# learning-at-home/dalle

Hardware: AMD Instinct MI355X
Metric: training samples/sec (whole node), DALL-E d_model=1024 at 1/2/4/8 MI355X (higher is better)
Workload: dtype bf16; 1 GPU; model=DALL-E d_model=1024, 24 layers, 256 text + 32x32 image tokens, preset=bench24, global_batch=128, per_gpu_batch=128, seq_len=1280, parallelism=dp1, unique_params=125648484, engine=GradSync + fused LAMB, optimizer=LAMB (32-bit moments) + global clip 4.0, grad_allreduce_dtype=fp32, grad_allreduce_algo=rccl, gemm_selection=off, reversible=no, grad_compression=none

## Files before the change

csrc/kernels/attention.hip:

```cpp
#include <cstdio>
#include <cstdlib>

#include "common.h"
#include <stdlib.h>
#include "geom.h"

#include "attn_tile.h"

namespace dalle {

__device__ __forceinline__ void rope_bwd_store_full(const RopeOut& ro, const AttnGeom& g, int bh, int s0, int t,
                                                    const f32x16& acc0, const f32x16& acc1, float scale, float* stage,
                                                    int lane) {
  const int hl = lane >> 5, c32 = lane & 31;
  const int b = bh / g.H, h = bh - b * g.H, HD = g.H * 64;
  const int q8 = lane & 7, d0 = 8 * q8;
  int pp[4];
  f32x4 c0[2], c1[2], n0[2], n1[2];
  auto load_tab = [&](int it) {
    const int tok = it * 8 + (lane >> 3);
    const int p = st2seq(g, s0 + tok);
    pp[it] = p;
    const int pc = p < 0 ? 0 : p;
    const float* cp = ro.cosT + (size_t)pc * 64 + d0;
    const float* sp = ro.sinT + (size_t)pc * 64 + d0;
    c0[it & 1] = *reinterpret_cast<const f32x4*>(cp);
    c1[it & 1] = *reinterpret_cast<const f32x4*>(cp + 4);
    n0[it & 1] = *reinterpret_cast<const f32x4*>(sp);
    n1[it & 1] = *reinterpret_cast<const f32x4*>(sp + 4);
  };
  load_tab(0);
  load_tab(1);
#pragma unroll
  for (int dt = 0; dt < 2; ++dt) {
    const f32x16& acc = dt ? acc1 : acc0;
#pragma unroll
    for (int gq = 0; gq < 4; ++gq) {
      const int ch = (8 * dt + 2 * gq + hl) ^ (c32 & 15);
      *reinterpret_cast<f32x4*>(stage + c32 * 64 + 4 * ch) = f32x4{acc[4 * gq], acc[4 * gq + 1], acc[4 * gq + 2], acc[4 * gq + 3]};
    }
  }
  __builtin_amdgcn_s_waitcnt(0xC07F);
  __builtin_amdgcn_wave_barrier();
#pragma unroll
  for (int it = 0; it < 4; ++it) {
    const int tok = it * 8 + (lane >> 3), sl = it & 1;
    const f32x4 lo = *reinterpret_cast<const f32x4*>(stage + tok * 64 + 4 * ((2 * q8) ^ (tok & 15)));
    const f32x4 hi = *reinterpret_cast<const f32x4*>(stage + tok * 64 + 4 * ((2 * q8 + 1) ^ (tok & 15)));
    const float x[8] = {lo[0], lo[1], lo[2], lo[3], hi[0], hi[1], hi[2], hi[3]};
    const float c[8] = {c0[sl][0], c0[sl][1], c0[sl][2], c0[sl][3], c1[sl][0], c1[sl][1], c1[sl][2], c1[sl][3]};
    const float sn[8] = {n0[sl][0], n0[sl][1], n0[sl][2], n0[sl][3], n1[sl][0], n1[sl][1], n1[sl][2], n1[sl][3]};
    const int p = pp[it];
    if (it + 2 < 4) load_tab(it + 2);
    float y[8];
#pragma unroll
    for (int i = 0; i < 8; i += 2) {
      const float a0 = x[i] * scale, a1 = x[i + 1] * scale;
      y[i] = a0 * c[i] + a1 * sn[i + 1];
      y[i + 1] = a1 * c[i + 1] + a0 * sn[i];
    }
    if (p >= 0) *reinterpret_cast<s16x8*>(ro.dqkv + ((size_t)b * g.n + p) * (3 * HD) + t * HD + h * 64 + d0) = pack8(y);
  }
  __builtin_amdgcn_wave_barrier();
}

constexpr float RESCALE_THR = 8.0f;

__device__ __forceinline__ float half_max(float x) {
  const auto r = __builtin_amdgcn_permlane32_swap(__float_as_uint(x), __float_as_uint(x), false, false);
  return fmaxf(__uint_as_float(r[0]), __uint_as_float(r[1]));
}
__device__ __forceinline__ float half_sum(float x) {
  const auto r = __builtin_amdgcn_permlane32_swap(__float_as_uint(x), __float_as_uint(x), false, false);
  return __uint_as_float(r[0]) + __uint_as_float(r[1]);
}

struct SoftmaxState {
  float m = NEG_BIG;
  float lsum = 0.f;
  f32x16 o0 = {}, o1 = {};
};

template <int NT>
__device__ __forceinline__ void fwd_tiles(SoftmaxState& st, const __bf16* const (&Ks)[NT], const __bf16* const (&Vs)[NT],
                                          const int (&kt)[NT], const bf16x8 (&qf)[4], const AttnGeom& g, int qb, int qs,
                                          int lane) {
  const int hl = lane >> 5, c32 = lane & 31;
  constexpr float THR_RAW = RESCALE_THR / LOG2E;
  f32x16 s[NT];
#pragma unroll
  for (int j = 0; j < NT; ++j) {
    s[j] = f32x16{};
#pragma unroll
    for (int ss = 0; ss < 4; ++ss) s[j] = MFMA32(row_operand(Ks[j], ss, c32, hl), qf[ss], s[j]);
// ... 128 lines not shown
        const int c = lane + 64 * j, row = c >> 3, col = (c & 7) * 8;
        *reinterpret_cast<s16x8*>(P + lds_idx(row, col)) = kr[j];
        *reinterpret_cast<s16x8*>(P + TILE + lds_idx(row, col)) = vr[j];
      }
      if (t < qb) load_loc(t + 1);
      __builtin_amdgcn_s_waitcnt(0xC07F);
      __builtin_amdgcn_wave_barrier();
      const __bf16* const Ks[1] = {P};
      const __bf16* const Vs[1] = {P + TILE};
      const int kt[1] = {t};
      fwd_tiles<1>(st, Ks, Vs, kt, qf, g, qb, qs, lane);
      __builtin_amdgcn_wave_barrier();
    }
  }

  if (!active) return;
  const float ltot = half_sum(st.lsum);
  const float inv = 1.0f / ltot;
  lse[(size_t)bh * g.Np + qs] = st.m * LOG2E + log2f(ltot);
  __bf16* Os = smem + wave * (2 * TILE);
#pragma unroll
  for (int dt = 0; dt < 2; ++dt) {
    const f32x16& o = dt ? st.o1 : st.o0;
#pragma unroll
    for (int gq = 0; gq < 4; ++gq) {
      float f[4];
#pragma unroll
      for (int i = 0; i < 4; ++i) f[i] = o[4 * gq + i] * inv;
      *reinterpret_cast<s16x4*>(Os + lds_idx(c32, 32 * dt + 8 * gq + 4 * hl)) = pack4(f);
    }
  }
  __builtin_amdgcn_s_waitcnt(0xC07F);
  __builtin_amdgcn_wave_barrier();
#pragma unroll
  for (int i = 0; i < 4; ++i) {
    const int row = 8 * i + (lane >> 3), col = (lane & 7) * 8;
    const s16x8 v = *reinterpret_cast<const s16x8*>(Os + lds_idx(row, col));
    const int p = st2seq(g, qb * 32 + row);
    if (p >= 0) *reinterpret_cast<s16x8*>(out + ((size_t)b * g.n + p) * (g.H * 64) + h * 64 + col) = v;
  }
}

__global__ __launch_bounds__(256) void attn_delta_kernel(const __bf16* __restrict__ dout, const __bf16* __restrict__ out,
                                                         float* __restrict__ delta, AttnGeom g, int BH) {
  const long gid = (long)blockIdx.x * blockDim.x + threadIdx.x;
  const int chunk = gid & 7;
  const long row_g = gid >> 3;
  if (row_g >= (long)BH * g.Np) return;
  const int bh = row_g / g.Np, srow = row_g - (long)bh * g.Np;
  const int off = tok_row(g, srow);
  float acc = 0.f;
  if (off >= 0) {
    float fd[8], fo[8];
    unpack8(ld_tok(tok_base(dout, g, bh), off, chunk * 8), fd);
    unpack8(ld_tok(tok_base(out, g, bh), off, chunk * 8), fo);
#pragma unroll
    for (int i = 0; i < 8; ++i) acc = fmaf(fd[i], fo[i], acc);
  }
  acc += __shfl_xor(acc, 1, 64);
  acc += __shfl_xor(acc, 2, 64);
  acc += __shfl_xor(acc, 4, 64);
  if (chunk == 0) delta[row_g] = acc;
}

__device__ __forceinline__ void dq_tile(f32x16& dq0, f32x16& dq1, const __bf16* Ks, const __bf16* Vs, int tile,
                                        const bf16x8 (&qf)[4], const bf16x8 (&dof)[4], float lq, float dl,
                                        const AttnGeom& g, int qb, int qs, int lane) {
  const int hl = lane >> 5, c32 = lane & 31;
  f32x16 s = {}, dp = {};
#pragma unroll
  for (int ss = 0; ss < 4; ++ss) {
    s = MFMA32(row_operand(Ks, ss, c32, hl), qf[ss], s);
    dp = MFMA32(row_operand(Vs, ss, c32, hl), dof[ss], dp);
  }
#pragma unroll
  for (int r = 0; r < 16; ++r) s[r] = fast_exp2(fmaf(s[r], LOG2E, -lq)) * (dp[r] - dl);
  if (!tile_full(g, qb, tile)) {
    const uint32_t mh = key_mask(g, qs, tile) >> (4 * hl);
#pragma unroll
    for (int r = 0; r < 16; ++r) s[r] = mask_bit(mh, r) ? s[r] : 0.f;
  }
  const bf16x8 d0 = cvt8(s, 0), d1 = cvt8(s, 8);
  dq0 = MFMA32(tr_operand(Ks, 0, 0, lane), d0, dq0);
  dq0 = MFMA32(tr_operand(Ks, 1, 0, lane), d1, dq0);
  dq1 = MFMA32(tr_operand(Ks, 0, 1, lane), d0, dq1);
  dq1 = MFMA32(tr_operand(Ks, 1, 1, lane), d1, dq1);
}

template <int MINB, bool FUSE_LOCAL, bool PREFETCH_LOCAL = false>
__global__ __launch_bounds__(256, MINB) void attn_bwd_dq_kernel(const __bf16* __restrict__ Q, const __bf16* __restrict__ Kt,
                                                             const __bf16* __restrict__ V, const __bf16* __restrict__ dout,
                                                             const __bf16* __restrict__ out, const float* __restrict__ lse,
                                                             float* __restrict__ delta, __bf16* __restrict__ dQ, AttnGeom g,
                                                             RopeOut ro, int delta_ready) {
  __shared__ __attribute__((aligned(16))) __bf16 smem[2 * 2 * 2 * TILE];
  __shared__ float fstats[FUSE_LOCAL ? 4 : 1][2][32];
  __shared__ float dsh[4][32];
  int grp, bh;
  xcd_remap(grp, bh);
  const int tid = threadIdx.x, wave = tid >> 6, lane = tid & 63, hl = lane >> 5;
  const int nqb = g.Np >> 5, ntext = g.Tp >> 5;
  const int qb0 = grp * 4;
  const int qb = qb0 + wave;
  const int qb_last = min(qb0 + 3, nqb - 1);
  const bool active = qb < nqb;
  const size_t base = (size_t)bh * g.Np * 64;
  const __bf16* dob = tok_base(dout, g, bh);
  const __bf16* outb = tok_base(out, g, bh);

  const int n_text = qb_last < ntext ? qb_last + 1 : ntext;
  const int my_text_end = active ? min(qb + 1, ntext) : 0;
  const int qs = qb * 32 + (lane & 31);
  const int qrow = active ? qs : 0;
  bf16x8 qf[4], dof[4];
  float dl = 0.f;
  {
  __bf16* Ps = smem + wave * (2 * TILE);
  float dpart[4];
  s16x8 qv[4], dv[4], ov[4];
  int toff[4];
#pragma unroll
  for (int j = 0; j < 4; ++j) {
    const int c = lane + 64 * j, row = c >> 3, col = (c & 7) * 8;
    const int srow = (active ? qb * 32 : 0) + row;
    toff[j] = tok_row(g, srow);
    const int safe = toff[j] < 0 ? 0 : toff[j];
    qv[j] = *reinterpret_cast<const s16x8*>(Q + base + (size_t)srow * 64 + col);
    dv[j] = *reinterpret_cast<const s16x8*>(dob + safe + col);
    ov[j] = *reinterpret_cast<const s16x8*>(outb + safe + col);
  }
#pragma unroll
  for (int j = 0; j < 4; ++j) {
    const int c = lane + 64 * j, row = c >> 3, col = (c & 7) * 8;
    if (toff[j] < 0) dv[j] = s16x8{};
    *reinterpret_cast<s16x8*>(Ps + lds_idx(row, col)) = qv[j];
    *reinterpret_cast<s16x8*>(Ps + TILE + lds_idx(row, col)) = dv[j];
    float fd[8], fo[8];
    unpack8(dv[j], fd);
    unpack8(ov[j], fo);
    dpart[j] = 0.f;
#pragma unroll
    for (int i = 0; i < 8; ++i) dpart[j] = fmaf(fd[i], fo[i], dpart[j]);
  }
  if (!delta_ready) {
#pragma unroll
    for (int j = 0; j < 4; ++j) {
      dpart[j] += __shfl_xor(dpart[j], 1, 64);
      dpart[j] += __shfl_xor(dpart[j], 2, 64);
      dpart[j] += __shfl_xor(dpart[j], 4, 64);
      const int row = 8 * j + (lane >> 3);
      if ((lane & 7) == 0) {
        dsh[wave][row] = dpart[j];
        if (active) delta[(size_t)bh * g.Np + qb * 32 + row] = dpart[j];
      }
    }
  }
  __builtin_amdgcn_s_waitcnt(0xC07F);
  __builtin_amdgcn_wave_barrier();
#pragma unroll
  for (int s2 = 0; s2 < 4; ++s2) {
    qf[s2] = row_operand(Ps, s2, lane & 31, hl);
    dof[s2] = row_operand(Ps + TILE, s2, lane & 31, hl);
  }
  dl = delta_ready ? delta[(size_t)bh * g.Np + qrow] : dsh[wave][lane & 31];
  __builtin_amdgcn_s_waitcnt(0xC07F);
  __syncthreads();
  }
  const float lq = lse[(size_t)bh * g.Np + qrow];
  f32x16 dq0 = {}, dq1 = {};
  const bool has_local = active && qb >= ntext;
  const int lo = has_local ? local_lo_tile(g, qb) : 0;
  s16x8 kr[4], vr[4];
  auto load_loc = [&](int t) {
#pragma unroll
    for (int j = 0; j < 4; ++j) {
      const int c = lane + 64 * j, row = c >> 3, col = (c & 7) * 8;
      const size_t off = base + (size_t)(t * 32 + row) * 64 + col;
      kr[j] = *reinterpret_cast<const s16x8*>(Kt + off);
      vr[j] = *reinterpret_cast<const s16x8*>(V + off);
    }
  };
  if (has_local && PREFETCH_LOCAL) load_loc(lo);

  {
  const int st_row = tid >> 3, st_col = (tid & 7) * 8;
  const int st_off = lds_idx(st_row, st_col);
  const int npairs = (n_text + 1) >> 1;
  s16x8 sreg[4];
  auto load_pair = [&](int pi) {
// ... 12 lines not shown
  };
  load_pair(0);
  store_pair(0);
  __syncthreads();
  for (int pi = 0; pi < npairs; ++pi) {
    const bool more = pi + 1 < npairs;
    if (more) load_pair(pi + 1);
    const __bf16* S0 = smem + (pi & 1) * (4 * TILE);
    const int ta = 2 * pi, tb = 2 * pi + 1;
    if (ta < my_text_end) dq_tile(dq0, dq1, S0, S0 + 2 * TILE, ta, qf, dof, lq, dl, g, qb, qs, lane);
    if (tb < my_text_end) dq_tile(dq0, dq1, S0 + TILE, S0 + 3 * TILE, tb, qf, dof, lq, dl, g, qb, qs, lane);
    if (more) store_pair((pi + 1) & 1);
    __syncthreads();
  }
  }

  if (has_local) {
    __bf16* P = smem + wave * (2 * TILE);
    if (!PREFETCH_LOCAL) load_loc(lo);
    for (int t = lo; t <= qb; ++t) {
#pragma unroll
      for (int j = 0; j < 4; ++j) {
        const int c = lane + 64 * j, row = c >> 3, col = (c & 7) * 8;
        *reinterpret_cast<s16x8*>(P + lds_idx(row, col)) = kr[j];
        *reinterpret_cast<s16x8*>(P + TILE + lds_idx(row, col)) = vr[j];
      }
      if (t < qb) load_loc(t + 1);
      __builtin_amdgcn_s_waitcnt(0xC07F);
      __builtin_amdgcn_wave_barrier();
      dq_tile(dq0, dq1, P, P + TILE, t, qf, dof, lq, dl, g, qb, qs, lane);
      __builtin_amdgcn_wave_barrier();
    }
  }
  if (FUSE_LOCAL && active && qb >= ntext && ro.dqkv) {
    __bf16* P = smem + wave * (2 * TILE);
    const int c32 = lane & 31;
    bf16x8 kf[4], vf[4];
#pragma unroll
    for (int s2 = 0; s2 < 4; ++s2) {
      kf[s2] = ld16(P + lds_idx(c32, 16 * s2 + 8 * hl));
      vf[s2] = ld16(P + TILE + lds_idx(c32, 16 * s2 + 8 * hl));
    }
    __builtin_amdgcn_s_waitcnt(0xC07F);
    __builtin_amdgcn_wave_barrier();
#pragma unroll
    for (int s2 = 0; s2 < 4; ++s2) {
      *reinterpret_cast<bf16x8*>(P + lds_idx(c32, 16 * s2 + 8 * hl)) = qf[s2];
      *reinterpret_cast<bf16x8*>(P + TILE + lds_idx(c32, 16 * s2 + 8 * hl)) = dof[s2];
    }
    if (hl == 0) {
      fstats[FUSE_LOCAL ? wave : 0][0][c32] = lq;
      fstats[FUSE_LOCAL ? wave : 0][1][c32] = dl;
    }
    __builtin_amdgcn_s_waitcnt(0xC07F);
    __builtin_amdgcn_wave_barrier();
    const float(*st)[32] = fstats[FUSE_LOCAL ? wave : 0];
    const int ks = qb * 32 + c32;
    f32x16 sc = {}, dp = {};
#pragma unroll
    for (int s2 = 0; s2 < 4; ++s2) {
      sc = MFMA32(row_operand(P, s2, c32, hl), kf[s2], sc);
      dp = MFMA32(row_operand(P + TILE, s2, c32, hl), vf[s2], dp);
    }
    f32x16 ds;
#pragma unroll
    for (int r = 0; r < 16; ++r) {
      const int ql = acc_row(r, hl);
      const float pr = fast_exp2(fmaf(sc[r], LOG2E, -st[0][ql]));
      sc[r] = pr;
      ds[r] = pr * (dp[r] - st[1][ql]);
    }
    const uint32_t mh = query_mask(g, ks, qb) >> (4 * hl);
#pragma unroll
    for (int r = 0; r < 16; ++r) {
      const bool on = mask_bit(mh, r);
      sc[r] = on ? sc[r] : 0.f;
      ds[r] = on ? ds[r] : 0.f;
    }
    const bf16x8 p0 = cvt8(sc, 0), p1 = cvt8(sc, 8);
    const bf16x8 e0 = cvt8(ds, 0), e1 = cvt8(ds, 8);
    f32x16 dk0 = {}, dk1 = {}, dv0 = {}, dv1 = {};
    dv0 = MFMA32(tr_operand(P + TILE, 0, 0, lane), p0, dv0);
    dv0 = MFMA32(tr_operand(P + TILE, 1, 0, lane), p1, dv0);
    dv1 = MFMA32(tr_operand(P + TILE, 0, 1, lane), p0, dv1);
    dv1 = MFMA32(tr_operand(P + TILE, 1, 1, lane), p1, dv1);
    dk0 = MFMA32(tr_operand(P, 0, 0, lane), e0, dk0);
    dk0 = MFMA32(tr_operand(P, 1, 0, lane), e1, dk0);
    dk1 = MFMA32(tr_operand(P, 0, 1, lane), e0, dk1);
    dk1 = MFMA32(tr_operand(P, 1, 1, lane), e1, dk1);
    float* stage = reinterpret_cast<float*>(P);
    rope_bwd_store_full(ro, g, bh, qb * 32, 1, dk0, dk1, 1.0f, stage, lane);
    rope_bwd_store_full(ro, g, bh, qb * 32, 2, dv0, dv1, 1.0f, stage, lane);
  }
  __syncthreads();

  if (!active) return;
  if (ro.dqkv) {
    float* stage = reinterpret_cast<float*>(smem) + wave * 2048;
    rope_bwd_store_full(ro, g, bh, qb * 32, 0, dq0, dq1, ro.qscale, stage, lane);
    return;
  }
  __bf16* qp = dQ + base + (size_t)qs * 64;
#pragma unroll
  for (int dt = 0; dt < 2; ++dt) {
    const f32x16& o = dt ? dq1 : dq0;
#pragma unroll
    for (int gq = 0; gq < 4; ++gq) {
      float f[4];
#pragma unroll
      for (int i = 0; i < 4; ++i) f[i] = o[4 * gq + i];
      *reinterpret_cast<s16x4*>(qp + 32 * dt + 8 * gq + 4 * hl) = pack4(f);
    }
  }
}

template <int MINB>
__global__ __launch_bounds__(256, MINB) void attn_bwd_dkdv_kernel(const __bf16* __restrict__ Q, const __bf16* __restrict__ Kt,
                                                               const __bf16* __restrict__ V, const __bf16* __restrict__ dout,
                                                               const float* __restrict__ lse, const float* __restrict__ delta,
                                                               __bf16* __restrict__ dK, __bf16* __restrict__ dV, AttnGeom g,
                                                               RopeOut ro) {
  __shared__ __attribute__((aligned(16))) __bf16 smem[4 * 2 * TILE];
  __shared__ float stats[4][2][32];
  int grp, bh;
  xcd_remap(grp, bh);
  const int tid = threadIdx.x, wave = tid >> 6, lane = tid & 63, hl = lane >> 5, c32 = lane & 31;
  const int nkb = g.Np >> 5, ntext = g.Tp >> 5;
  const int kb = ntext + grp * 4 + wave;
  if (kb >= nkb) return;
  const size_t base = (size_t)bh * g.Np * 64;
  const __bf16* dob = tok_base(dout, g, bh);
  const int ks = kb * 32 + c32;
  const int q_hi = local_hi_qtile(g, kb);
  bf16x8 kf[4], vf[4];
  {
    const __bf16* kp = Kt + base + (size_t)ks * 64 + 8 * hl;
    const __bf16* vp = V + base + (size_t)ks * 64 + 8 * hl;
#pragma unroll
    for (int s = 0; s < 4; ++s) { kf[s] = ld16(kp + 16 * s); vf[s] = ld16(vp + 16 * s); }
  }
  __bf16* Qs = smem + wave * (2 * TILE);
  __bf16* Ds = Qs + TILE;
  s16x8 qr[4], dr[4];
  float sv = 0.f;
  auto load_tile = [&](int qt) {
#pragma unroll
    for (int j = 0; j < 4; ++j) {
      const int c = lane + 64 * j, row = c >> 3, col = (c & 7) * 8;
      const size_t off = base + (size_t)(qt * 32 + row) * 64 + col;
      qr[j] = *reinterpret_cast<const s16x8*>(Q + off);
      dr[j] = ld_tok(dob, tok_row(g, qt * 32 + row), col);
    }
    sv = (hl ? delta : lse)[(size_t)bh * g.Np + qt * 32 + c32];
  };
  f32x16 dk0 = {}, dk1 = {}, dv0 = {}, dv1 = {};
  load_tile(kb);
  for (int qt = kb; qt <= q_hi; ++qt) {
#pragma unroll
    for (int j = 0; j < 4; ++j) {
      const int c = lane + 64 * j, row = c >> 3, col = (c & 7) * 8;
      *reinterpret_cast<s16x8*>(Qs + lds_idx(row, col)) = qr[j];
      *reinterpret_cast<s16x8*>(Ds + lds_idx(row, col)) = dr[j];
    }
    stats[wave][hl][c32] = sv;
    if (qt < q_hi) load_tile(qt + 1);
    __builtin_amdgcn_s_waitcnt(0xC07F);
    __builtin_amdgcn_wave_barrier();
    f32x16 sc = {}, dp = {};
#pragma unroll
    for (int ss = 0; ss < 4; ++ss) {
      sc = MFMA32(row_operand(Qs, ss, c32, hl), kf[ss], sc);
      dp = MFMA32(row_operand(Ds, ss, c32, hl), vf[ss], dp);
    }
    f32x16 ds;
#pragma unroll
    for (int r = 0; r < 16; ++r) {
      const int ql = acc_row(r, hl);
      const float pr = fast_exp2(fmaf(sc[r], LOG2E, -stats[wave][0][ql]));
      sc[r] = pr;
      ds[r] = pr * (dp[r] - stats[wave][1][ql]);
    }
    if (!tile_full(g, qt, kb)) {
      const uint32_t mh = query_mask(g, ks, qt) >> (4 * hl);
#pragma unroll
      for (int r = 0; r < 16; ++r) {
        const bool on = mask_bit(mh, r);
        sc[r] = on ? sc[r] : 0.f;
        ds[r] = on ? ds[r] : 0.f;
      }
    }
    const bf16x8 p0 = cvt8(sc, 0), p1 = cvt8(sc, 8);
    const bf16x8 d0 = cvt8(ds, 0), d1 = cvt8(ds, 8);
    dv0 = MFMA32(tr_operand(Ds, 0, 0, lane), p0, dv0);
    dv0 = MFMA32(tr_operand(Ds, 1, 0, lane), p1, dv0);
    dv1 = MFMA32(tr_operand(Ds, 0, 1, lane), p0, dv1);
    dv1 = MFMA32(tr_operand(Ds, 1, 1, lane), p1, dv1);
    dk0 = MFMA32(tr_operand(Qs, 0, 0, lane), d0, dk0);
    dk0 = MFMA32(tr_operand(Qs, 1, 0, lane), d1, dk0);
    dk1 = MFMA32(tr_operand(Qs, 0, 1, lane), d0, dk1);
    dk1 = MFMA32(tr_operand(Qs, 1, 1, lane), d1, dk1);
    __builtin_amdgcn_wave_barrier();
  }
  if (ro.dqkv) {
    float* stage = reinterpret_cast<float*>(Qs);
    rope_bwd_store_full(ro, g, bh, kb * 32, 1, dk0, dk1, 1.0f, stage, lane);
    rope_bwd_store_full(ro, g, bh, kb * 32, 2, dv0, dv1, 1.0f, stage, lane);
    return;
  }
  __bf16* kp = dK + base + (size_t)ks * 64;
  __bf16* vp = dV + base + (size_t)ks * 64;
#pragma unroll
  for (int dt = 0; dt < 2; ++dt) {
    const f32x16& a = dt ? dk1 : dk0;
    const f32x16& c = dt ? dv1 : dv0;
#pragma unroll
    for (int gq = 0; gq < 4; ++gq) {
      float fa[4], fc[4];
#pragma unroll
      for (int i = 0; i < 4; ++i) { fa[i] = a[4 * gq + i]; fc[i] = c[4 * gq + i]; }
      *reinterpret_cast<s16x4*>(kp + 32 * dt + 8 * gq + 4 * hl) = pack4(fa);
      *reinterpret_cast<s16x4*>(vp + 32 * dt + 8 * gq + 4 * hl) = pack4(fc);
    }
  }
}

template <int MINB, int QT = 2>
__global__ __launch_bounds__(256, MINB) void attn_bwd_dkdv_text_kernel(const __bf16* __restrict__ Q, const __bf16* __restrict__ Kt,
                                                                    const __bf16* __restrict__ V, const __bf16* __restrict__ dout,
                                                                    const float* __restrict__ lse, const float* __restrict__ delta,
                                                                    __bf16* __restrict__ dK, __bf16* __restrict__ dV, AttnGeom g,
                                                                    RopeOut ro) {
  static_assert(QT == 2 || QT == 4, "QT");
  __shared__ __attribute__((aligned(16))) __bf16 smem[2 * QT * 2 * TILE];
  __shared__ float stats[2][QT][2][32];
  int grp, bh;
  xcd_remap(grp, bh);
  const int tid = threadIdx.x, wave = tid >> 6, lane = tid & 63, hl = lane >> 5, c32 = lane & 31;
  const int nqb = g.Np >> 5, ntext = g.Tp >> 5;
  const int kb0 = grp * 2;
  const bool tail = QT == 4 && kb0 + 1 >= ntext;
  const int kb = tail ? kb0 : kb0 + (wave & 1), par = tail ? wave : wave >> 1;
  const bool active = kb < ntext;
  const size_t base = (size_t)bh * g.Np * 64;
  const __bf16* dob = tok_base(dout, g, bh);
  const int ks = kb * 32 + c32;
  bf16x8 kf[4], vf[4];
  {
    const int krow = active ? ks : 0;
    const __bf16* kp = Kt + base + (size_t)krow * 64 + 8 * hl;
    const __bf16* vp = V + base + (size_t)krow * 64 + 8 * hl;
#pragma unroll
    for (int s = 0; s < 4; ++s) { kf[s] = ld16(kp + 16 * s); vf[s] = ld16(vp + 16 * s); }
  }
  const int nsteps = (nqb - kb0 + QT - 1) / QT;
  const int st_row = (tid & 255) >> 3, st_col = (tid & 7) * 8;
  const int st_off = lds_idx(st_row, st_col);
  s16x8 sreg[2 * QT];
  float sl = 0.f;
  auto load_step = [&](int i) {
#pragma unroll
    for (int pp = 0; pp < QT; ++pp) {
      const int qt = min(kb0 + QT * i + pp, nqb - 1);
      const size_t off = base + (size_t)(qt * 32 + st_row) * 64 + st_col;
      sreg[2 * pp] = *reinterpret_cast<const s16x8*>(Q + off);
      sreg[2 * pp + 1] = ld_tok(dob, tok_row(g, qt * 32 + st_row), st_col);
    }
    if (tid < QT * 64) {
      const int pp = tid >> 6, which = (tid >> 5) & 1, r = tid & 31;
      const int qt = min(kb0 + QT * i + pp, nqb - 1);
      const float* src = which ? delta : lse;
      sl = src[(size_t)bh * g.Np + qt * 32 + r];
    }
  };
  auto store_step = [&](int buf) {
#pragma unroll
    for (int pp = 0; pp < QT; ++pp) {
      __bf16* T0 = smem + (buf * QT + pp) * (2 * TILE);
      *reinterpret_cast<s16x8*>(T0 + st_off) = sreg[2 * pp];
      *reinterpret_cast<s16x8*>(T0 + TILE + st_off) = sreg[2 * pp + 1];
    }
    if (tid < QT * 64) stats[buf][tid >> 6][(tid >> 5) & 1][tid & 31] = sl;
  };
  f32x16 dk0 = {}, dk1 = {}, dv0 = {}, dv1 = {};
  if (nsteps > 0) {
    load_step(0);
    store_step(0);
  }
  __builtin_amdgcn_s_waitcnt(0x0F70);
  __syncthreads();
  auto scores = [&](const __bf16* Qs, const __bf16* Ds, f32x16& sc, f32x16& dp) {
    sc = f32x16{};
    dp = f32x16{};
#pragma unroll
    for (int ss = 0; ss < 4; ++ss) {
      sc = MFMA32(row_operand(Qs, ss, c32, hl), kf[ss], sc);
      dp = MFMA32(row_operand(Ds, ss, c32, hl), vf[ss], dp);
    }
  };
  auto probs = [&](int buf, int tt, int qt, f32x16& sc, f32x16& dp) {
#pragma unroll
    for (int r = 0; r < 16; ++r) {
      const int ql = acc_row(r, hl);
      const float pr = fast_exp2(fmaf(sc[r], LOG2E, -stats[buf][tt][0][ql]));
      sc[r] = pr;
      dp[r] = pr * (dp[r] - stats[buf][tt][1][ql]);
    }
    if (!tile_full(g, qt, kb)) {
      const uint32_t mh = query_mask(g, ks, qt) >> (4 * hl);
#pragma unroll
      for (int r = 0; r < 16; ++r) {
        const bool on = mask_bit(mh, r);
        sc[r] = on ? sc[r] : 0.f;
        dp[r] = on ? dp[r] : 0.f;
      }
    }
  };
  auto accum = [&](const __bf16* Qs, const __bf16* Ds, const f32x16& sc, const f32x16& ds) {
    const bf16x8 p0 = cvt8(sc, 0), p1 = cvt8(sc, 8);
    const bf16x8 d0 = cvt8(ds, 0), d1 = cvt8(ds, 8);
    dv0 = MFMA32(tr_operand(Ds, 0, 0, lane), p0, dv0);
    dv0 = MFMA32(tr_operand(Ds, 1, 0, lane), p1, dv0);
    dv1 = MFMA32(tr_operand(Ds, 0, 1, lane), p0, dv1);
    dv1 = MFMA32(tr_operand(Ds, 1, 1, lane), p1, dv1);
    dk0 = MFMA32(tr_operand(Qs, 0, 0, lane), d0, dk0);
    dk0 = MFMA32(tr_operand(Qs, 1, 0, lane), d1, dk0);
    dk1 = MFMA32(tr_operand(Qs, 0, 1, lane), d0, dk1);
    dk1 = MFMA32(tr_operand(Qs, 1, 1, lane), d1, dk1);
  };
  for (int i = 0; i < nsteps; ++i) {
    const bool more = i + 1 < nsteps;
    if (more) load_step(i + 1);
    const int buf = i & 1;
#pragma unroll
    for (int u = 0; u < QT / 2; ++u) {
      const int tt = tail ? par : par + 2 * u;
      const int qt = kb0 + QT * i + tt;
      if (active && qt < nqb && qt >= kb && !(tail && u > 0)) {
        const __bf16* Qs = smem + (buf * QT + tt) * (2 * TILE);
        f32x16 sc, dp;
        scores(Qs, Qs + TILE, sc, dp);
        probs(buf, tt, qt, sc, dp);
        accum(Qs, Qs + TILE, sc, dp);
      }
    }
    if (more) store_step((i + 1) & 1);
    __syncthreads();
  }
  float* red = reinterpret_cast<float*>(smem);
  if (par != 0) {
    const int slot = tail ? wave - 1 : (wave & 1);
#pragma unroll
    for (int r = 0; r < 16; ++r) {
      red[(slot * 64 + r) * 64 + lane] = dk0[r];
      red[(slot * 64 + 16 + r) * 64 + lane] = dk1[r];
      red[(slot * 64 + 32 + r) * 64 + lane] = dv0[r];
      red[(slot * 64 + 48 + r) * 64 + lane] = dv1[r];
    }
  }
  __syncthreads();
  if (par == 0 && active) {
    const int s0 = tail ? 0 : (wave & 1), s1 = tail ? 3 : s0 + 1;
    for (int sl2 = s0; sl2 < s1; ++sl2) {
      const float* mine = red + sl2 * 64 * 64;
#pragma unroll
      for (int r = 0; r < 16; ++r) {
        dk0[r] += mine[r * 64 + lane];
        dk1[r] += mine[(16 + r) * 64 + lane];
        dv0[r] += mine[(32 + r) * 64 + lane];
        dv1[r] += mine[(48 + r) * 64 + lane];
      }
    }
    if (ro.dqkv) {
      __builtin_amdgcn_s_waitcnt(0xC07F);
      __builtin_amdgcn_wave_barrier();
      float* stage = red + (wave & 1) * 64 * 64;
      rope_bwd_store_full(ro, g, bh, kb * 32, 1, dk0, dk1, 1.0f, stage, lane);
      rope_bwd_store_full(ro, g, bh, kb * 32, 2, dv0, dv1, 1.0f, stage, lane);
    } else {
      __bf16* kp = dK + base + (size_t)ks * 64;
      __bf16* vp = dV + base + (size_t)ks * 64;
#pragma unroll
      for (int dt = 0; dt < 2; ++dt) {
        const f32x16& a = dt ? dk1 : dk0;
        const f32x16& c = dt ? dv1 : dv0;
#pragma unroll
        for (int gq = 0; gq < 4; ++gq) {
          float fa[4], fc[4];
#pragma unroll
          for (int i = 0; i < 4; ++i) {
            fa[i] = a[4 * gq + i];
            fc[i] = c[4 * gq + i];
          }
          *reinterpret_cast<s16x4*>(kp + 32 * dt + 8 * gq + 4 * hl) = pack4(fa);
          *reinterpret_cast<s16x4*>(vp + 32 * dt + 8 * gq + 4 * hl) = pack4(fc);
        }
      }
    }
  }
}

void attn_fwd(const void* q, const void* k, const void* v, void* out, float* lse, const AttnGeom& g, int BH, hipStream_t st) {
  dim3 grid((g.Np / 32 + 3) / 4, BH);
  hipLaunchKernelGGL((attn_fwd_kernel<3, false>), grid, dim3(256), 0, st, (const __bf16*)q, (const __bf16*)k,
                     (const __bf16*)v, (__bf16*)out, lse, g);
}

bool attn_bwd_fused_ok(const AttnGeom& g, bool rope_out, bool has_freqs);
void attn_bwd_fused_launch(const void* q, const void* k, const void* v, const void* dout, const void* out, const float* lse,
                           const AttnGeom& g, int BH, hipStream_t st, const RopeOut& ro, const RotSpec& rsp);

void attn_bwd(const void* q, const void* k, const void* v, const void* out, const void* dout, const float* lse,
              float* delta, void* dq, void* dk, void* dv, const AttnGeom& g, int BH, hipStream_t st,
              const float* cosT, const float* sinT, void* dqkv, float qscale, const float* rotf, int rot_nl, int rot_np,
              float rot_img_text_pos, float rot_text_axial) {
  const RopeOut ro{cosT, sinT, static_cast<__bf16*>(dqkv), qscale};
  if (attn_bwd_fused_ok(g, dqkv != nullptr, rotf != nullptr)) {
    attn_bwd_fused_launch(q, k, v, dout, out, lse, g, BH, st, ro, RotSpec{rotf, rot_nl, rot_np, rot_img_text_pos, rot_text_axial});
    return;
  }
  dim3 grid((g.Np / 32 + 3) / 4, BH);
  const bool fuse_local = dqkv != nullptr && (g.pattern == 1 || g.pattern == 2);
  const int ntext = g.Tp / 32, nimg = g.Np / 32 - ntext;
  if (fuse_local)
    hipLaunchKernelGGL((attn_bwd_dq_kernel<3, true, false>), grid, dim3(256), 0, st, (const __bf16*)q, (const __bf16*)k,
                       (const __bf16*)v, (const __bf16*)dout, (const __bf16*)out, lse, delta, (__bf16*)dq, g, ro, 0);
  else
    hipLaunchKernelGGL((attn_bwd_dq_kernel<3, false, false>), grid, dim3(256), 0, st, (const __bf16*)q, (const __bf16*)k,
                       (const __bf16*)v, (const __bf16*)dout, (const __bf16*)out, lse, delta, (__bf16*)dq, g, ro, 0);
  hipLaunchKernelGGL((attn_bwd_dkdv_text_kernel<2, 4>), dim3((ntext + 1) / 2, BH), dim3(256), 0, st, (const __bf16*)q,
                     (const __bf16*)k, (const __bf16*)v, (const __bf16*)dout, lse, delta, (__bf16*)dk, (__bf16*)dv, g, ro);
  if (!fuse_local)
    hipLaunchKernelGGL((attn_bwd_dkdv_kernel<2>), dim3((nimg + 3) / 4, BH), dim3(256), 0, st, (const __bf16*)q,
                       (const __bf16*)k, (const __bf16*)v, (const __bf16*)dout, lse, delta, (__bf16*)dk, (__bf16*)dv, g, ro);
}

}
```

csrc/kernels/attn_tile.h:

```cpp
#pragma once
#include "common.h"
#include "geom.h"

namespace dalle {

__device__ __forceinline__ int swz(int r) { return (((r >> 1) & 1) << 2) | ((r >> 2) & 3); }
__device__ __forceinline__ int lds_idx(int r, int col) { return r * 64 + ((((col >> 3) ^ swz(r)) << 3) | (col & 7)); }
constexpr int TILE = 32 * 64;

__device__ __forceinline__ void dma_tile(const __bf16* src_rows, __bf16* tile, int wave, int lane) {
  const int row = 8 * wave + (lane >> 3);
  const __bf16* gp = src_rows + (size_t)row * 64 + (((lane & 7) ^ swz(row)) << 3);
  __builtin_amdgcn_global_load_lds((const void __attribute__((address_space(1)))*)gp,
                                   (void __attribute__((address_space(3)))*)(tile + 512 * wave), 16, 0, 0);
}
__device__ __forceinline__ void dma_tile_wave(const __bf16* src_rows, __bf16* tile, int lane) {
#pragma unroll
  for (int piece = 0; piece < 4; ++piece) dma_tile(src_rows, tile, piece, lane);
}
constexpr int WAIT_VM0 = 0x0F70;

__device__ __forceinline__ float fast_exp2(float x) { return __builtin_amdgcn_exp2f(x); }

__device__ __forceinline__ int st2seq(const AttnGeom& g, int s) {
  if (s < g.T) return s;
  if (s < g.Tp) return -1;
  const int kst = s - g.Tp;
  const int k = (g.pattern == 2) ? ((kst & (g.S - 1)) << g.logS) + (kst >> g.logS) : kst;
  const int p = g.T + k;
  return p < g.n ? p : -1;
}

__device__ __forceinline__ const __bf16* tok_base(const __bf16* x, const AttnGeom& g, int bh) {
  const int b = bh / g.H, h = bh - b * g.H;
  return x + (size_t)b * g.n * (g.H * 64) + h * 64;
}
__device__ __forceinline__ int tok_row(const AttnGeom& g, int s) {
  const int k = s - g.Tp;
  const int kk = (g.pattern == 2) ? ((k & (g.S - 1)) << g.logS) + (k >> g.logS) : k;
  const int p = s < g.Tp ? (s < g.T ? s : -1) : (g.T + kk < g.n ? g.T + kk : -1);
  return p < 0 ? -1 : p * (g.H * 64);
}
__device__ __forceinline__ s16x8 ld_tok(const __bf16* __restrict__ xb, int row_off, int col) {
  return row_off < 0 ? s16x8{} : *reinterpret_cast<const s16x8*>(xb + row_off + col);
}

__device__ __forceinline__ uint32_t range_bits(int lo, int hi) {
  lo = max(lo, 0);
  hi = min(hi, 31);
  if (hi < lo) return 0u;
  const uint32_t upto = hi == 31 ? 0xffffffffu : ((1u << (hi + 1)) - 1u);
  return upto & ~((1u << lo) - 1u);
}

__device__ __forceinline__ uint32_t key_mask(const AttnGeom& g, int qs, int kt) {
  const int k0 = kt * 32;
  if (qs < g.Tp) return range_bits(0, qs - k0);
  if (k0 < g.Tp) return range_bits(0, g.T - 1 - k0);
  const int qk = qs - g.Tp, kk0 = k0 - g.Tp;
  if (g.pattern == 0) return range_bits(0, qk - kk0);
  const int qr = qk >> g.logS;
  if (g.pattern != 3) return range_bits((qr << g.logS) - kk0, qk - kk0);
  const int qc = qk & (g.S - 1);
  const int c_lo = max(0, qc - g.K + 1);
  const int rows = g.S >= 32 ? 1 : (32 >> g.logS);
  uint32_t m = 0u;
  for (int i = 0; i < rows; ++i) {
    const int kr = (kk0 >> g.logS) + i;
    if (kr > qr - g.K && kr <= qr) m |= range_bits((kr << g.logS) + c_lo - kk0, (kr << g.logS) + qc - kk0);
  }
  return m;
}

__device__ __forceinline__ uint32_t query_mask(const AttnGeom& g, int ks, int qt) {
  const int q0 = qt * 32;
  if (ks < g.Tp) {
    if (q0 < g.Tp) return range_bits(ks - q0, 31);
    return ks < g.T ? 0xffffffffu : 0u;
  }
  if (q0 < g.Tp) return 0u;
  const int kk = ks - g.Tp, qk0 = q0 - g.Tp;
  if (g.pattern == 0) return range_bits(kk - qk0, 31);
  const int kr = kk >> g.logS;
  if (g.pattern != 3) return range_bits(kk - qk0, ((kr + 1) << g.logS) - 1 - qk0);
  const int kc = kk & (g.S - 1);
  const int c_hi = min(g.S - 1, kc + g.K - 1);
  const int rows = g.S >= 32 ? 1 : (32 >> g.logS);
  uint32_t m = 0u;
  for (int i = 0; i < rows; ++i) {
    const int qr = (qk0 >> g.logS) + i;
    if (qr >= kr && qr < kr + g.K) m |= range_bits((qr << g.logS) + kc - qk0, (qr << g.logS) + c_hi - qk0);
  }
  return m;
}

__device__ __forceinline__ bool tile_full(const AttnGeom& g, int qt, int kt) {
  const int ntext = g.Tp >> 5;
  if (kt < ntext) {
    if (kt * 32 + 31 >= g.T) return false;
    return qt >= ntext || kt < qt;
  }
  return g.pattern == 0 && qt >= ntext && kt < qt;
}

__device__ __forceinline__ void xcd_remap(int& grp, int& bh) {
  const int ng = gridDim.x, BH = gridDim.y;
  if (BH & 7) { grp = blockIdx.x; bh = blockIdx.y; return; }
  const int L = blockIdx.x + blockIdx.y * ng;
  const int x = L & 7, j = L >> 3;
  bh = x + 8 * (j / ng);
  grp = j - (j / ng) * ng;
}

__device__ __forceinline__ int local_lo_tile(const AttnGeom& g, int qb) {
  const int kq0 = qb * 32 - g.Tp;
  int lo;
  if (g.pattern == 0) lo = 0;
  else if (g.pattern == 3) lo = max(0, (kq0 >> g.logS) - (g.K - 1)) << g.logS;
  else lo = (kq0 >> g.logS) << g.logS;
  return (g.Tp + lo) >> 5;
}

__device__ __forceinline__ int local_hi_qtile(const AttnGeom& g, int kb) {
  const int kk1 = kb * 32 + 31 - g.Tp;
// ... 58 lines not shown
```

Baseline: 318.6 samples/s.

## Precompute tile row positions and 32-bit byte offsets in attention backward kernels

Adds a TilePos/RopeRows helper that works out the sequence positions for a tile once, from a wave-uniform start, and stores precomputed 32-bit byte offsets. These replace the per-row st2seq/tok_row calls and 64-bit address arithmetic in the rope stores, the output writes and the dout loads. It also loads the Q tile by DMA in the dq kernel, applies the mask inside the exp so masked entries skip work, unrolls the mask loops with a fixed bound, and uses readfirstlane for wave-uniform values. A host check rejects shapes whose offsets would overflow 32 bits. The goal is lower integer/VALU and addressing overhead in the attention backward pass, which is only a small part of whole-step training.

```diff
diff --git a/csrc/kernels/attention.hip b/csrc/kernels/attention.hip
--- a/csrc/kernels/attention.hip
+++ b/csrc/kernels/attention.hip
@@ -1,5 +1,7 @@
 #include <cstdio>
 #include <cstdlib>
+#include <stdexcept>
+#include <string>
 
 #include "common.h"
 #include <stdlib.h>
@@ -9,57 +11,72 @@
 
 namespace dalle {
 
-__device__ __forceinline__ void rope_bwd_store_full(const RopeOut& ro, const AttnGeom& g, int bh, int s0, int t,
+struct RopeRows {
+  uint32_t tab[4];
+  uint32_t dst[4];
+};
+__device__ __forceinline__ RopeRows rope_rows(const AttnGeom& g, int s0, int lane) {
+  const TilePos tp = tile_pos(g, s0, lane);
+  const uint32_t q8 = lane & 7, row_bytes = 3u * g.H * 64u * 2u;
+  RopeRows rr;
+#pragma unroll
+  for (int it = 0; it < 4; ++it) {
+    const int p = tp.p[it];
+    rr.tab[it] = (uint32_t)(p < 0 ? 0 : p) * 256u + 32u * q8;
+    rr.dst[it] = p < 0 ? ~0u : (uint32_t)p * row_bytes + 16u * q8;
+  }
+  return rr;
+}
+
+template <bool SCALE>
+__device__ __forceinline__ void rope_bwd_store_full(const RopeOut& ro, const AttnGeom& g, int bh, int t, const RopeRows& rr,
                                                     const f32x16& acc0, const f32x16& acc1, float scale, float* stage,
                                                     int lane) {
   const int hl = lane >> 5, c32 = lane & 31;
   const int b = bh / g.H, h = bh - b * g.H, HD = g.H * 64;
-  const int q8 = lane & 7, d0 = 8 * q8;
-  int pp[4];
+  const int q8 = lane & 7, l3 = lane >> 3;
+  const char* cosb = reinterpret_cast<const char*>(ro.cosT);
+  const char* sinb = reinterpret_cast<const char*>(ro.sinT);
+  char* dstb = reinterpret_cast<char*>(ro.dqkv + ((size_t)b * g.n * 3 + t) * HD + h * 64);
   f32x4 c0[2], c1[2], n0[2], n1[2];
   auto load_tab = [&](int it) {
-    const int tok = it * 8 + (lane >> 3);
-    const int p = st2seq(g, s0 + tok);
-    pp[it] = p;
-    const int pc = p < 0 ? 0 : p;
-    const float* cp = ro.cosT + (size_t)pc * 64 + d0;
-    const float* sp = ro.sinT + (size_t)pc * 64 + d0;
+    const char* cp = cosb + rr.tab[it];
+    const char* sp = sinb + rr.tab[it];
     c0[it & 1] = *reinterpret_cast<const f32x4*>(cp);
-    c1[it & 1] = *reinterpret_cast<const f32x4*>(cp + 4);
+    c1[it & 1] = *reinterpret_cast<const f32x4*>(cp + 16);
     n0[it & 1] = *reinterpret_cast<const f32x4*>(sp);
-    n1[it & 1] = *reinterpret_cast<const f32x4*>(sp + 4);
+    n1[it & 1] = *reinterpret_cast<const f32x4*>(sp + 16);
   };
   load_tab(0);
   load_tab(1);
+  const int wbase = c32 * 64 + 4 * (hl ^ (c32 & 15));
 #pragma unroll
   for (int dt = 0; dt < 2; ++dt) {
     const f32x16& acc = dt ? acc1 : acc0;
 #pragma unroll
-    for (int gq = 0; gq < 4; ++gq) {
-      const int ch = (8 * dt + 2 * gq + hl) ^ (c32 & 15);
-      *reinterpret_cast<f32x4*>(stage + c32 * 64 + 4 * ch) = f32x4{acc[4 * gq], acc[4 * gq + 1], acc[4 * gq + 2], acc[4 * gq + 3]};
-    }
+    for (int gq = 0; gq < 4; ++gq)
+      *reinterpret_cast<f32x4*>(stage + (wbase ^ (4 * (8 * dt + 2 * gq)))) = f32x4{acc[4 * gq], acc[4 * gq + 1], acc[4 * gq + 2], acc[4 * gq + 3]};
   }
   __builtin_amdgcn_s_waitcnt(0xC07F);
   __builtin_amdgcn_wave_barrier();
+  const int rbase = l3 * 64 + 4 * ((2 * q8) ^ l3);
 #pragma unroll
   for (int it = 0; it < 4; ++it) {
-    const int tok = it * 8 + (lane >> 3), sl = it & 1;
-    const f32x4 lo = *reinterpret_cast<const f32x4*>(stage + tok * 64 + 4 * ((2 * q8) ^ (tok & 15)));
-    const f32x4 hi = *reinterpret_cast<const f32x4*>(stage + tok * 64 + 4 * ((2 * q8 + 1) ^ (tok & 15)));
+    const int sl = it & 1, rd = it * 512 + (rbase ^ (32 * (it & 1)));
+    const f32x4 lo = *reinterpret_cast<const f32x4*>(stage + rd);
+    const f32x4 hi = *reinterpret_cast<const f32x4*>(stage + (rd ^ 4));
     const float x[8] = {lo[0], lo[1], lo[2], lo[3], hi[0], hi[1], hi[2], hi[3]};
     const float c[8] = {c0[sl][0], c0[sl][1], c0[sl][2], c0[sl][3], c1[sl][0], c1[sl][1], c1[sl][2], c1[sl][3]};
     const float sn[8] = {n0[sl][0], n0[sl][1], n0[sl][2], n0[sl][3], n1[sl][0], n1[sl][1], n1[sl][2], n1[sl][3]};
-    const int p = pp[it];
     if (it + 2 < 4) load_tab(it + 2);
     float y[8];
 #pragma unroll
     for (int i = 0; i < 8; i += 2) {
-      const float a0 = x[i] * scale, a1 = x[i + 1] * scale;
+      const float a0 = SCALE ? x[i] * scale : x[i], a1 = SCALE ? x[i + 1] * scale : x[i + 1];
       y[i] = a0 * c[i] + a1 * sn[i + 1];
       y[i + 1] = a1 * c[i + 1] + a0 * sn[i];
     }
-    if (p >= 0) *reinterpret_cast<s16x8*>(ro.dqkv + ((size_t)b * g.n + p) * (3 * HD) + t * HD + h * 64 + d0) = pack8(y);
+    if (rr.dst[it] != ~0u) *reinterpret_cast<s16x8*>(dstb + rr.dst[it]) = pack8(y);
   }
   __builtin_amdgcn_wave_barrier();
 }
@@ -254,12 +271,14 @@
   }
   __builtin_amdgcn_s_waitcnt(0xC07F);
   __builtin_amdgcn_wave_barrier();
+  const TilePos tp = tile_pos(g, qb * 32, lane);
+  char* ob = reinterpret_cast<char*>(out + (size_t)b * g.n * (g.H * 64) + h * 64);
+  const uint32_t row_bytes = g.H * 64 * 2;
 #pragma unroll
   for (int i = 0; i < 4; ++i) {
     const int row = 8 * i + (lane >> 3), col = (lane & 7) * 8;
     const s16x8 v = *reinterpret_cast<const s16x8*>(Os + lds_idx(row, col));
-    const int p = st2seq(g, qb * 32 + row);
-    if (p >= 0) *reinterpret_cast<s16x8*>(out + ((size_t)b * g.n + p) * (g.H * 64) + h * 64 + col) = v;
+    if (tp.p[i] >= 0) *reinterpret_cast<s16x8*>(ob + ((uint32_t)tp.p[i] * row_bytes + 2 * col)) = v;
   }
 }
 
@@ -318,9 +337,13 @@
   __shared__ __attribute__((aligned(16))) __bf16 smem[2 * 2 * 2 * TILE];
   __shared__ float fstats[FUSE_LOCAL ? 4 : 1][2][32];
   __shared__ float dsh[4][32];
+  if (FUSE_LOCAL) {
+    __builtin_assume(g.pattern == 1 || g.pattern == 2);
+    __builtin_assume(ro.dqkv != nullptr);
+  }
   int grp, bh;
   xcd_remap(grp, bh);
-  const int tid = threadIdx.x, wave = tid >> 6, lane = tid & 63, hl = lane >> 5;
+  const int tid = threadIdx.x, wave = __builtin_amdgcn_readfirstlane(tid >> 6), lane = tid & 63, hl = lane >> 5;
   const int nqb = g.Np >> 5, ntext = g.Tp >> 5;
   const int qb0 = grp * 4;
   const int qb = qb0 + wave;
@@ -339,23 +362,22 @@
   {
   __bf16* Ps = smem + wave * (2 * TILE);
   float dpart[4];
-  s16x8 qv[4], dv[4], ov[4];
-  int toff[4];
+  s16x8 dv[4], ov[4];
+  const int srow0 = active ? qb * 32 : 0;
+  dma_tile_wave(Q + base + (size_t)srow0 * 64, Ps, lane);
+  const TilePos tp = tile_pos(g, srow0, lane);
+  const uint32_t row_bytes = g.H * 64 * 2;
+#pragma unroll
+  for (int j = 0; j < 4; ++j) {
+    const uint32_t off = (uint32_t)max(tp.p[j], 0) * row_bytes + 16 * (lane & 7);
+    dv[j] = *reinterpret_cast<const s16x8*>(reinterpret_cast<const char*>(dob) + off);
+    ov[j] = *reinterpret_cast<const s16x8*>(reinterpret_cast<const char*>(outb) + off);
+  }
+  __builtin_amdgcn_sched_barrier(0);
 #pragma unroll
   for (int j = 0; j < 4; ++j) {
     const int c = lane + 64 * j, row = c >> 3, col = (c & 7) * 8;
-    const int srow = (active ? qb * 32 : 0) + row;
-    toff[j] = tok_row(g, srow);
-    const int safe = toff[j] < 0 ? 0 : toff[j];
-    qv[j] = *reinterpret_cast<const s16x8*>(Q + base + (size_t)srow * 64 + col);
-    dv[j] = *reinterpret_cast<const s16x8*>(dob + safe + col);
-    ov[j] = *reinterpret_cast<const s16x8*>(outb + safe + col);
-  }
-#pragma unroll
-  for (int j = 0; j < 4; ++j) {
-    const int c = lane + 64 * j, row = c >> 3, col = (c & 7) * 8;
-    if (toff[j] < 0) dv[j] = s16x8{};
-    *reinterpret_cast<s16x8*>(Ps + lds_idx(row, col)) = qv[j];
+    if (tp.p[j] < 0) dv[j] = s16x8{};
     *reinterpret_cast<s16x8*>(Ps + TILE + lds_idx(row, col)) = dv[j];
     float fd[8], fo[8];
     unpack8(dv[j], fd);
@@ -364,19 +386,18 @@
 #pragma unroll
     for (int i = 0; i < 8; ++i) dpart[j] = fmaf(fd[i], fo[i], dpart[j]);
   }
-  if (!delta_ready) {
-#pragma unroll
-    for (int j = 0; j < 4; ++j) {
-      dpart[j] += __shfl_xor(dpart[j], 1, 64);
-      dpart[j] += __shfl_xor(dpart[j], 2, 64);
-      dpart[j] += __shfl_xor(dpart[j], 4, 64);
-      const int row = 8 * j + (lane >> 3);
-      if ((lane & 7) == 0) {
-        dsh[wave][row] = dpart[j];
-        if (active) delta[(size_t)bh * g.Np + qb * 32 + row] = dpart[j];
-      }
-    }
-  }
+#pragma unroll
+  for (int j = 0; j < 4; ++j) {
+    dpart[j] += __shfl_xor(dpart[j], 1, 64);
+    dpart[j] += __shfl_xor(dpart[j], 2, 64);
+    dpart[j] += __shfl_xor(dpart[j], 4, 64);
+    const int row = 8 * j + (lane >> 3);
+    if ((lane & 7) == 0) {
+      dsh[wave][row] = dpart[j];
+      if (!delta_ready && active) delta[(size_t)bh * g.Np + qb * 32 + row] = dpart[j];
+    }
+  }
+  __builtin_amdgcn_s_waitcnt(WAIT_VM0);
   __builtin_amdgcn_s_waitcnt(0xC07F);
   __builtin_amdgcn_wave_barrier();
 #pragma unroll
@@ -455,9 +476,11 @@
       __builtin_amdgcn_wave_barrier();
     }
   }
+  RopeRows rr = {};
+  if (active && ro.dqkv) rr = rope_rows(g, qb * 32, fresh_lane());
   if (FUSE_LOCAL && active && qb >= ntext && ro.dqkv) {
     __bf16* P = smem + wave * (2 * TILE);
-    const int c32 = lane & 31;
+    const int lane = fresh_lane(), hl = lane >> 5, c32 = lane & 31;
     bf16x8 kf[4], vf[4];
 #pragma unroll
     for (int s2 = 0; s2 < 4; ++s2) {
@@ -485,20 +508,14 @@
       sc = MFMA32(row_operand(P, s2, c32, hl), kf[s2], sc);
       dp = MFMA32(row_operand(P + TILE, s2, c32, hl), vf[s2], dp);
     }
+    const uint32_t mh = query_mask(g, ks, qb) >> (4 * hl);
     f32x16 ds;
 #pragma unroll
     for (int r = 0; r < 16; ++r) {
       const int ql = acc_row(r, hl);
-      const float pr = fast_exp2(fmaf(sc[r], LOG2E, -st[0][ql]));
+      const float pr = mask_bit(mh, r) ? fast_exp2(fmaf(sc[r], LOG2E, -st[0][ql])) : 0.f;
       sc[r] = pr;
       ds[r] = pr * (dp[r] - st[1][ql]);
-    }
-    const uint32_t mh = query_mask(g, ks, qb) >> (4 * hl);
-#pragma unroll
-    for (int r = 0; r < 16; ++r) {
-      const bool on = mask_bit(mh, r);
-      sc[r] = on ? sc[r] : 0.f;
-      ds[r] = on ? ds[r] : 0.f;
     }
     const bf16x8 p0 = cvt8(sc, 0), p1 = cvt8(sc, 8);
     const bf16x8 e0 = cvt8(ds, 0), e1 = cvt8(ds, 8);
@@ -512,15 +529,15 @@
     dk1 = MFMA32(tr_operand(P, 0, 1, lane), e0, dk1);
     dk1 = MFMA32(tr_operand(P, 1, 1, lane), e1, dk1);
     float* stage = reinterpret_cast<float*>(P);
-    rope_bwd_store_full(ro, g, bh, qb * 32, 1, dk0, dk1, 1.0f, stage, lane);
-    rope_bwd_store_full(ro, g, bh, qb * 32, 2, dv0, dv1, 1.0f, stage, lane);
+    rope_bwd_store_full<false>(ro, g, bh, 1, rr, dk0, dk1, 1.0f, stage, lane);
+    rope_bwd_store_full<false>(ro, g, bh, 2, rr, dv0, dv1, 1.0f, stage, lane);
   }
   __syncthreads();
 
   if (!active) return;
   if (ro.dqkv) {
     float* stage = reinterpret_cast<float*>(smem) + wave * 2048;
-    rope_bwd_store_full(ro, g, bh, qb * 32, 0, dq0, dq1, ro.qscale, stage, lane);
+    rope_bwd_store_full<true>(ro, g, bh, 0, rr, dq0, dq1, ro.qscale, stage, fresh_lane());
     return;
   }
   __bf16* qp = dQ + base + (size_t)qs * 64;
@@ -547,7 +564,7 @@
   __shared__ float stats[4][2][32];
   int grp, bh;
   xcd_remap(grp, bh);
-  const int tid = threadIdx.x, wave = tid >> 6, lane = tid & 63, hl = lane >> 5, c32 = lane & 31;
+  const int tid = threadIdx.x, wave = __builtin_amdgcn_readfirstlane(tid >> 6), lane = tid & 63, hl = lane >> 5, c32 = lane & 31;
   const int nkb = g.Np >> 5, ntext = g.Tp >> 5;
   const int kb = ntext + grp * 4 + wave;
   if (kb >= nkb) return;
@@ -566,13 +583,17 @@
   __bf16* Ds = Qs + TILE;
   s16x8 qr[4], dr[4];
   float sv = 0.f;
+  const uint32_t row_bytes = g.H * 64 * 2;
   auto load_tile = [&](int qt) {
+    const TilePos tp = tile_pos(g, qt * 32, lane);
 #pragma unroll
     for (int j = 0; j < 4; ++j) {
       const int c = lane + 64 * j, row = c >> 3, col = (c & 7) * 8;
       const size_t off = base + (size_t)(qt * 32 + row) * 64 + col;
       qr[j] = *reinterpret_cast<const s16x8*>(Q + off);
-      dr[j] = ld_tok(dob, tok_row(g, qt * 32 + row), col);
+      dr[j] = s16x8{};
+      if (tp.p[j] >= 0)
+        dr[j] = *reinterpret_cast<const s16x8*>(reinterpret_cast<const char*>(dob) + ((uint32_t)tp.p[j] * row_bytes + 2 * col));
     }
     sv = (hl ? delta : lse)[(size_t)bh * g.Np + qt * 32 + c32];
   };
@@ -595,23 +616,16 @@
       sc = MFMA32(row_operand(Qs, ss, c32, hl), kf[ss], sc);
       dp = MFMA32(row_operand(Ds, ss, c32, hl), vf[ss], dp);
     }
-    f32x16 ds;
-#pragma unroll
-    for (int r = 0; r < 16; ++r) {
-      const int ql = acc_row(r, hl);
-      const float pr = fast_exp2(fmaf(sc[r], LOG2E, -stats[wave][0][ql]));
-      sc[r] = pr;
-      ds[r] = pr * (dp[r] - stats[wave][1][ql]);
-    }
+#pragma unroll
+    for (int r = 0; r < 16; ++r) sc[r] = fast_exp2(fmaf(sc[r], LOG2E, -stats[wave][0][acc_row(r, hl)]));
     if (!tile_full(g, qt, kb)) {
       const uint32_t mh = query_mask(g, ks, qt) >> (4 * hl);
 #pragma unroll
-      for (int r = 0; r < 16; ++r) {
-        const bool on = mask_bit(mh, r);
-        sc[r] = on ? sc[r] : 0.f;
-        ds[r] = on ? ds[r] : 0.f;
-      }
-    }
+      for (int r = 0; r < 16; ++r) sc[r] = mask_bit(mh, r) ? sc[r] : 0.f;
+    }
+    f32x16 ds;
+#pragma unroll
+    for (int r = 0; r < 16; ++r) ds[r] = sc[r] * (dp[r] - stats[wave][1][acc_row(r, hl)]);
     const bf16x8 p0 = cvt8(sc, 0), p1 = cvt8(sc, 8);
     const bf16x8 d0 = cvt8(ds, 0), d1 = cvt8(ds, 8);
     dv0 = MFMA32(tr_operand(Ds, 0, 0, lane), p0, dv0);
@@ -626,8 +640,9 @@
   }
   if (ro.dqkv) {
     float* stage = reinterpret_cast<float*>(Qs);
-    rope_bwd_store_full(ro, g, bh, kb * 32, 1, dk0, dk1, 1.0f, stage, lane);
-    rope_bwd_store_full(ro, g, bh, kb * 32, 2, dv0, dv1, 1.0f, stage, lane);
+    const RopeRows rr = rope_rows(g, kb * 32, lane);
+    rope_bwd_store_full<false>(ro, g, bh, 1, rr, dk0, dk1, 1.0f, stage, lane);
+    rope_bwd_store_full<false>(ro, g, bh, 2, rr, dv0, dv1, 1.0f, stage, lane);
     return;
   }
   __bf16* kp = dK + base + (size_t)ks * 64;
@@ -658,7 +673,7 @@
   __shared__ float stats[2][QT][2][32];
   int grp, bh;
   xcd_remap(grp, bh);
-  const int tid = threadIdx.x, wave = tid >> 6, lane = tid & 63, hl = lane >> 5, c32 = lane & 31;
+  const int tid = threadIdx.x, wave = __builtin_amdgcn_readfirstlane(tid >> 6), lane = tid & 63, hl = lane >> 5, c32 = lane & 31;
   const int nqb = g.Np >> 5, ntext = g.Tp >> 5;
   const int kb0 = grp * 2;
   const bool tail = QT == 4 && kb0 + 1 >= ntext;
@@ -680,13 +695,17 @@
   const int st_off = lds_idx(st_row, st_col);
   s16x8 sreg[2 * QT];
   float sl = 0.f;
+  const uint32_t row_bytes = g.H * 64 * 2;
   auto load_step = [&](int i) {
 #pragma unroll
     for (int pp = 0; pp < QT; ++pp) {
       const int qt = min(kb0 + QT * i + pp, nqb - 1);
       const size_t off = base + (size_t)(qt * 32 + st_row) * 64 + st_col;
       sreg[2 * pp] = *reinterpret_cast<const s16x8*>(Q + off);
-      sreg[2 * pp + 1] = ld_tok(dob, tok_row(g, qt * 32 + st_row), st_col);
+      const int p = tile_row_pos(g, qt * 32, st_row);
+      sreg[2 * pp + 1] = s16x8{};
+      if (p >= 0)
+        sreg[2 * pp + 1] = *reinterpret_cast<const s16x8*>(reinterpret_cast<const char*>(dob) + ((uint32_t)p * row_bytes + 2 * st_col));
     }
     if (tid < QT * 64) {
       const int pp = tid >> 6, which = (tid >> 5) & 1, r = tid & 31;
@@ -722,21 +741,14 @@
   };
   auto probs = [&](int buf, int tt, int qt, f32x16& sc, f32x16& dp) {
 #pragma unroll
-    for (int r = 0; r < 16; ++r) {
-      const int ql = acc_row(r, hl);
-      const float pr = fast_exp2(fmaf(sc[r], LOG2E, -stats[buf][tt][0][ql]));
-      sc[r] = pr;
-      dp[r] = pr * (dp[r] - stats[buf][tt][1][ql]);
-    }
+    for (int r = 0; r < 16; ++r) sc[r] = fast_exp2(fmaf(sc[r], LOG2E, -stats[buf][tt][0][acc_row(r, hl)]));
     if (!tile_full(g, qt, kb)) {
       const uint32_t mh = query_mask(g, ks, qt) >> (4 * hl);
 #pragma unroll
-      for (int r = 0; r < 16; ++r) {
-        const bool on = mask_bit(mh, r);
-        sc[r] = on ? sc[r] : 0.f;
-        dp[r] = on ? dp[r] : 0.f;
-      }
-    }
+      for (int r = 0; r < 16; ++r) sc[r] = mask_bit(mh, r) ? sc[r] : 0.f;
+    }
+#pragma unroll
+    for (int r = 0; r < 16; ++r) dp[r] = sc[r] * (dp[r] - stats[buf][tt][1][acc_row(r, hl)]);
   };
   auto accum = [&](const __bf16* Qs, const __bf16* Ds, const f32x16& sc, const f32x16& ds) {
     const bf16x8 p0 = cvt8(sc, 0), p1 = cvt8(sc, 8);
@@ -797,8 +809,9 @@
       __builtin_amdgcn_s_waitcnt(0xC07F);
       __builtin_amdgcn_wave_barrier();
       float* stage = red + (wave & 1) * 64 * 64;
-      rope_bwd_store_full(ro, g, bh, kb * 32, 1, dk0, dk1, 1.0f, stage, lane);
-      rope_bwd_store_full(ro, g, bh, kb * 32, 2, dv0, dv1, 1.0f, stage, lane);
+      const RopeRows rr = rope_rows(g, kb * 32, lane);
+      rope_bwd_store_full<false>(ro, g, bh, 1, rr, dk0, dk1, 1.0f, stage, lane);
+      rope_bwd_store_full<false>(ro, g, bh, 2, rr, dv0, dv1, 1.0f, stage, lane);
     } else {
       __bf16* kp = dK + base + (size_t)ks * 64;
       __bf16* vp = dV + base + (size_t)ks * 64;
@@ -822,7 +835,15 @@
   }
 }
 
+static void check_extents(const AttnGeom& g, int BH, const char* who) {
+  const long long elems = (long long)(BH / g.H) * g.n * 3 * g.H * 64, tab_bytes = (long long)(g.n + 1) * 64 * 4;
+  if (elems >= (1ll << 31) || tab_bytes >= (1ll << 31))
+    throw std::runtime_error(std::string(who) + ": B * n * 3 * H * 64 = " + std::to_string(elems) +
+                             " elements (or the rotary tables) exceed the kernels' 32-bit offsets");
+}
+
 void attn_fwd(const void* q, const void* k, const void* v, void* out, float* lse, const AttnGeom& g, int BH, hipStream_t st) {
+  check_extents(g, BH, "attn_fwd");
   dim3 grid((g.Np / 32 + 3) / 4, BH);
   hipLaunchKernelGGL((attn_fwd_kernel<3, false>), grid, dim3(256), 0, st, (const __bf16*)q, (const __bf16*)k,
                      (const __bf16*)v, (__bf16*)out, lse, g);
@@ -836,6 +857,7 @@
               float* delta, void* dq, void* dk, void* dv, const AttnGeom& g, int BH, hipStream_t st,
               const float* cosT, const float* sinT, void* dqkv, float qscale, const float* rotf, int rot_nl, int rot_np,
               float rot_img_text_pos, float rot_text_axial) {
+  check_extents(g, BH, "attn_bwd");
   const RopeOut ro{cosT, sinT, static_cast<__bf16*>(dqkv), qscale};
   if (attn_bwd_fused_ok(g, dqkv != nullptr, rotf != nullptr)) {
     attn_bwd_fused_launch(q, k, v, dout, out, lse, g, BH, st, ro, RotSpec{rotf, rot_nl, rot_np, rot_img_text_pos, rot_text_axial});
diff --git a/csrc/kernels/attn_tile.h b/csrc/kernels/attn_tile.h
--- a/csrc/kernels/attn_tile.h
+++ b/csrc/kernels/attn_tile.h
@@ -43,6 +43,40 @@
 }
 __device__ __forceinline__ s16x8 ld_tok(const __bf16* __restrict__ xb, int row_off, int col) {
   return row_off < 0 ? s16x8{} : *reinterpret_cast<const s16x8*>(xb + row_off + col);
+}
+
+__device__ __forceinline__ int fresh_lane() { return __builtin_amdgcn_mbcnt_hi(~0u, __builtin_amdgcn_mbcnt_lo(~0u, 0u)); }
+
+struct TilePos {
+  int p[4];
+};
+__device__ __forceinline__ int tile_row_pos(const AttnGeom& g, int s0, int row) {
+  s0 = __builtin_amdgcn_readfirstlane(s0);
+  if (s0 < g.Tp) return s0 + row < g.T ? s0 + row : -1;
+  const int kst = s0 - g.Tp + row;
+  const int k = (g.pattern == 2) ? ((kst & (g.S - 1)) << g.logS) + (kst >> g.logS) : kst;
+  return g.T + k < g.n ? g.T + k : -1;
+}
+__device__ __forceinline__ TilePos tile_pos(const AttnGeom& g, int s0, int lane) {
+  s0 = __builtin_amdgcn_readfirstlane(s0);
+  const int r = lane >> 3;
+  TilePos tp;
+  if (s0 < g.Tp) {
+#pragma unroll
+    for (int it = 0; it < 4; ++it) {
+      const int s = s0 + 8 * it + r;
+      tp.p[it] = s < g.T ? s : -1;
+    }
+  } else {
+    const int k0 = s0 - g.Tp + r;
+#pragma unroll
+    for (int it = 0; it < 4; ++it) {
+      const int kst = k0 + 8 * it;
+      const int k = (g.pattern == 2) ? ((kst & (g.S - 1)) << g.logS) + (kst >> g.logS) : kst;
+      tp.p[it] = g.T + k < g.n ? g.T + k : -1;
+    }
+  }
+  return tp;
 }
 
 __device__ __forceinline__ uint32_t range_bits(int lo, int hi) {
@@ -65,9 +99,10 @@
   const int c_lo = max(0, qc - g.K + 1);
   const int rows = g.S >= 32 ? 1 : (32 >> g.logS);
   uint32_t m = 0u;
-  for (int i = 0; i < rows; ++i) {
+#pragma unroll
+  for (int i = 0; i < 4; ++i) {
     const int kr = (kk0 >> g.logS) + i;
-    if (kr > qr - g.K && kr <= qr) m |= range_bits((kr << g.logS) + c_lo - kk0, (kr << g.logS) + qc - kk0);
+    if (i < rows && kr > qr - g.K && kr <= qr) m |= range_bits((kr << g.logS) + c_lo - kk0, (kr << g.logS) + qc - kk0);
   }
   return m;
 }
@@ -87,9 +122,10 @@
   const int c_hi = min(g.S - 1, kc + g.K - 1);
   const int rows = g.S >= 32 ? 1 : (32 >> g.logS);
   uint32_t m = 0u;
-  for (int i = 0; i < rows; ++i) {
+#pragma unroll
+  for (int i = 0; i < 4; ++i) {
     const int qr = (qk0 >> g.logS) + i;
-    if (qr >= kr && qr < kr + g.K) m |= range_bits((qr << g.logS) + kc - qk0, (qr << g.logS) + c_hi - qk0);
+    if (i < rows && qr >= kr && qr < kr + g.K) m |= range_bits((qr << g.logS) + kc - qk0, (qr << g.logS) + c_hi - qk0);
   }
   return m;
 }
```

Measured after the change: 320.8 samples/s, median of 6. About the same (+0.7%).
